# zfountas/deep-active-inference-mc

Measured on AMD Instinct MI355X. Metric: EFE rollouts/sec (64x64 dSprites, 10 MC-samples, depth 5), higher is better.
Workload: dtype f32; 1 GPU; calculate_G_repeated: 128 rows (32 roots x 4 actions) x depth 5 x 10 MC samples per GPU (BASELINE configs[1]) + action posterior; rows_per_gpu=128, samples=10, depth=5, parallelism=episodes sharded x1, weights replicated

## Files before the change

deep-active-inference-mc_amd/csrc/decoder.hip:

```cpp
#include "mfma_pipe.h"

namespace efe {

constexpr int DA_PS = 17;
constexpr int DA_BIAS = 257 * DA_PS;

__host__ __device__ constexpr int wino_i0(int a) { return a == 0 ? 0 : (a == 2 ? 2 : 1); }
__host__ __device__ constexpr int wino_i1(int a) { return a == 0 ? 2 : (a == 1 ? 2 : (a == 2 ? 1 : 3)); }
__host__ __device__ constexpr float wino_s1(int a) { return a == 1 ? 1.0f : -1.0f; }
__host__ __device__ constexpr float wino_at(int r, int a) { return r == 0 ? (a < 3 ? 1.0f : 0.0f) : (a == 0 ? 0.0f : (a == 1 ? 1.0f : -1.0f)); }

template <int NR, int R0, class Pix>
__device__ __forceinline__ void wino_l1(f32x16 (&out)[NR][2], const float4* __restrict__ U, const float4* sm, const int h,
                                        const int mt_, Pix pix) {
    constexpr int PD = 4;
    const unsigned ln = (threadIdx.x & 63u) * 16u;
    const __amdgpu_buffer_rsrc_t ur = wrsrc(U);
    int mt = mt_; asm volatile("" : "+s"(mt));
    constexpr int a_lo = NR == 2 ? 0 : R0, a_hi = NR == 2 ? 4 : R0 + 3;
    auto ufrag = [&](int a, int b, int kc) { return wfrag(ur, ln, (size_t)(((4 * a + b) * 2 + mt) * 8 + kc) * 64); };
    auto bases = [&](int a, int b, int (&pb)[4]) {
        const int i0 = wino_i0(a), i1 = wino_i1(a), j0 = wino_i0(b), j1 = wino_i1(b);
        pb[0] = pix(i0, j0); pb[1] = pix(i0, j1); pb[2] = pix(i1, j0); pb[3] = pix(i1, j1);
    };
    float4 aq[PD], raw[4];
    int pb[4];
#pragma unroll
    for (int p = 0; p < PD; ++p) aq[p] = ufrag(a_lo, 0, p);
    bases(a_lo, 0, pb);
#pragma unroll
    for (int q = 0; q < 4; ++q) raw[q] = sm[pb[q] + h];
    f32x16 xacc;
    const f32x16 zero = {};
    auto otrans = [&](int a, int b, const f32x16& m, auto mask) {
        constexpr int MASK = decltype(mask)::value;
#pragma unroll
        for (int r = 0; r < NR; ++r) {
            if (!((MASK >> r) & 1)) continue;
            const float car = wino_at(R0 + r, a);
#pragma unroll
            for (int c = 0; c < 2; ++c) {
                const float cbc = wino_at(c, b);
                if (cbc == 0.0f) continue;
                const float cf = car * cbc;
#pragma unroll
                for (int e = 0; e < 16; ++e) out[r][c][e] = __builtin_fmaf(cf, m[e], out[r][c][e]);
            }
        }
    };
    auto xi_row = [&](int a, auto mask) {
        const float s1 = wino_s1(a);
        const int an = a + 1 < a_hi ? a + 1 : a;
// ... 215 lines not shown
            return ((unsigned)y < 16u && (unsigned)x < 16u ? sy * 16 + x : DAS_IN) * DA_PS;
        };
        if (r) wino_l1<1, 1>(o, W1, sin, h, mt, pix);
        else wino_l1<1, 0>(o, W1, sin, h, mt, pix);
        if (j < 16)
#pragma unroll
        for (int c = 0; c < 2; ++c)
#pragma unroll
            for (int g4 = 0; g4 < 4; ++g4) {
                float4 v;
                v.x = relu_bits(o[0][c][4 * g4 + 0]); v.y = relu_bits(o[0][c][4 * g4 + 1]);
                v.z = relu_bits(o[0][c][4 * g4 + 2]); v.w = relu_bits(o[0][c][4 * g4 + 3]);
                sl1[((ly + 1 + r) * 16 + lx + 1 + c) * DA_PS + mt * 8 + 2 * g4 + h] = v;
            }
    }
    __syncthreads();
    float* Y = a.y2 + (size_t)img * (32 * 32 * 64);
    const int vrows = min(4, 16 - 2 * p);
#pragma unroll 1
    for (int k = 0; k < 2; ++k) {
        const int par = (w & 1) ? (k ? 2 : 1) : (k ? 3 : 0);
        const int ph = par >> 1, pw = par & 1;
        acc_init(16);
        tap_loop_pd<1, 1, 2>(acc, (1 + ph) * (1 + pw), W2, sl1, h, ConvT2Addr<1, DA_PS>{ph, pw, j >> 4, 0, j & 15, vrows, 16, DAS_L1}, PackedWIdx{2, 8, mt});
        float4* yp = reinterpret_cast<float4*>(Y) + (size_t)par * 4096 + ((2 * p) * 16 + j) * 2 + h;
#pragma unroll
        for (int g4 = 0; g4 < 4; ++g4) {
            float4 v;
            v.x = relu_bits(acc[0][0][4 * g4 + 0]); v.y = relu_bits(acc[0][0][4 * g4 + 1]);
            v.z = relu_bits(acc[0][0][4 * g4 + 2]); v.w = relu_bits(acc[0][0][4 * g4 + 3]);
            yp[(mt * 4 + g4) * 512] = v;
        }
    }
}

constexpr size_t DA_LDS_BYTES = (257 * DA_PS + 33) * sizeof(float4);
int init_dec_b_kernels();
int init_decoder_kernels() {
    if (hipFuncSetAttribute((const void*)k_dec_a, hipFuncAttributeMaxDynamicSharedMemorySize, DA_LDS_BYTES) != hipSuccess) return 1;
    if (hipFuncSetAttribute((const void*)k_dec_a_s, hipFuncAttributeMaxDynamicSharedMemorySize, DAS_LDS_BYTES) != hipSuccess) return 1;
    return init_dec_b_kernels();
}

void launch_dec_a(const DecAArgs& a, hipStream_t st) {
    if (a.parts == 8) {
        hipLaunchKernelGGL(k_dec_a_s, dim3(a.rows * 8), dim3(256), DAS_LDS_BYTES, st, a);
        return;
    }
    const size_t lds = DA_LDS_BYTES;
    const int grid = a.rows < 512 ? a.rows : 512;
    hipLaunchKernelGGL(k_dec_a, dim3(grid), dim3(256), lds, st, a);
}

template <int PARTS>
__global__ void __launch_bounds__(256, 2) k_dec_b4(const DecBArgs a) {
    constexpr int SR = 4, NW = 4, NTHR = 256;
    constexpr int DB_ZERO = (SR + 1) * 32;
    constexpr int DB_PS = 17;
    constexpr int DB_IN_F4 = (DB_ZERO + 1) * DB_PS;
    constexpr int DB_YROWS = 4 * SR + 2;
    constexpr int NPF = (SR + 1) * 512 / NTHR;
    constexpr int NS = 32 / SR;
    extern __shared__ __attribute__((aligned(16))) float4 sm[];
    float* sH = reinterpret_cast<float*>(sm + DB_IN_F4);
    __shared__ float4 sb3[8];
    const int tid = threadIdx.x;
    const int lane = tid & 63;
    const int w = __builtin_amdgcn_readfirstlane(tid >> 6);
    const int j = lane & 31, h = lane >> 5;
    constexpr int parts = PARTS;
    const int img = parts == 1 ? (int)blockIdx.x : (int)(blockIdx.x >> 2);
    const int qtr = parts == 1 ? 0 : (int)(blockIdx.x & 3);
    if (!row_live(a.live, img)) return;
    const int s_lo = parts == 1 ? 0 : (qtr ? 2 * qtr - 1 : 0);
    const int s_hi = parts == 1 ? NS : 2 * qtr + 2;

    const int mg = a.m0 + img;
    const int g = mg / a.rows_per_group;
    const int r = mg - g * a.rows_per_group;
    int gt, gp, gs;
    group_decode(a.gm, g, gt, gp, gs);
    const int mode = (gp == 0 && a.reward0) ? 1 : 0;
    const int slot = (gp == 0 && a.store0) ? gt * a.gm.S + gs : -1;
    float* po = (slot >= 0) ? a.po + ((size_t)slot * a.rows_per_group + r) * 4096 : nullptr;

    __shared__ float sq[4 * NTHR];
    __shared__ float sQ[4];
    if (tid < 8) sb3[tid] = reinterpret_cast<const float4*>(a.b3)[tid];
    __shared__ float4 sW4[8 * 12];
    if (tid < 96) {
        const int pat = tid / 12, i4 = tid - pat * 12;
        const int kw = pat & 3, hh = pat >> 2, kh = i4 >> 2, g4 = i4 & 3;
        sW4[tid] = kw < 3 ? reinterpret_cast<const float4*>(a.w4 + (3 * kh + kw) * 32)[2 * g4 + hh] : make_float4(0.f, 0.f, 0.f, 0.f);
    }
    const float4* w4p = sW4 + (h * 4 + (lane & 3)) * 12;
    if (tid < 16) sm[DB_ZERO * DB_PS + tid] = make_float4(0.f, 0.f, 0.f, 0.f);

    const float4* X = reinterpret_cast<const float4*>(a.y2) + (size_t)img * (32 * 32 * 16);
    const float4* W3 = reinterpret_cast<const float4*>(a.w3);
    const __amdgpu_buffer_rsrc_t wr = wrsrc(W3);
    const unsigned ln = (unsigned)lane * 16u;
    const float D1 = 1.00001f, D0 = 0.00001f;
    float part = 0.f;
    f32x4 pf[NPF];
    f32x4* smv = reinterpret_cast<f32x4*>(sm);
    const f32x4* Xv = reinterpret_cast<const f32x4*>(X);
    auto y2_at = [&](int iy, int idx) -> size_t { return (size_t)(((iy & 1) * 16 + ((idx & 511) >> 5)) * 512 + (iy >> 1) * 32 + (idx & 31)); };
#pragma unroll
    for (int it = 0; it < NPF; ++it) { const int idx = it * NTHR + tid; pf[it] = Xv[y2_at(min(SR * s_lo + (idx >> 9), 31), idx)]; }

    const int spA = w * 32 + j;
    const int spB = (j < 31) ? w * 32 + j + 1 : DB_ZERO;
    const int spC = (w + 1) * 32 + j;
    const int spD = (j < 31) ? (w + 1) * 32 + j + 1 : DB_ZERO;
    auto wf = [&](int tap, int kc) -> float4 { return wfrag(wr, ln, (size_t)(tap * 8 + kc) * 64); };

    constexpr int RWG = 2 * SR / NW;
    float gh[RWG][6], gpr[RWG];
    auto g_load = [&](int oh, int q, int r0y, int hb0) {
#pragma unroll
        for (int kh = 0; kh < 3; ++kh) {
            const int tr = oh + 1 - kh;
            const bool rv = tr >= 0 && tr <= 63;
            int hs = hb0 + (tr - r0y);
            hs = hs < 0 ? hs + DB_YROWS : hs;
            hs = hs >= DB_YROWS ? hs - DB_YROWS : hs;
            hs = rv ? hs : 0;
            const float* hq = sH + ((hs * 2) * 3 + kh) * 64 + lane;
            gh[q][2 * kh] = hq[0]; gh[q][2 * kh + 1] = hq[3 * 64];
        }
    };
    auto g_sig = [&](int oh, int q) {
        float v = a.b4;
#pragma unroll
        for (int kh = 0; kh < 3; ++kh) {
            const int tr = oh + 1 - kh;
            v += (tr >= 0 && tr <= 63) ? gh[q][2 * kh] + gh[q][2 * kh + 1] : 0.f;
        }
        gpr[q] = hw_sigmoid(v);
    };
    auto g_term = [&](int oh, int q) {
#pragma clang fp contract(off)
        const float pr = gpr[q];
        const float l1 = hw_log(D1 - pr), l0 = hw_log(D0 + pr);
        const float te = __builtin_fmaf(pr - 1.0f, l1, -(pr * l0));
        const float tw = reward_term(pr, oh, lane, 64, 64, a.reward_intent);
        const float t = mode == 0 ? te : tw;
        part += oh >= 0 ? t : 0.0f;
    };
    auto g_store = [&](int oh, int q) {
        if (po && oh >= 0) {
            int owl = lane; asm volatile("" : "+v"(owl));
            (po + oh * 64)[owl] = gpr[q];
        }
    };
    auto prefetch = [&](int sn, int tl) {
#pragma unroll
        for (int it = 0; it < NPF; ++it) {
            const int idx = it * NTHR + tl;
            const int grow = min(SR * sn + (idx >> 9), 31);
            pf[it] = Xv[y2_at(grow, idx)];
        }
    };

    auto fold = [&](int k) { sq[k * NTHR + tid] = part; part = 0.f; };
    int hb = 0, hbp = 0;
    for (int s = s_lo; s < s_hi; ++s) {
        const int tl = tid;
        const bool gq = parts == 1 ? true : s == 2 * qtr + 1;
        const int oh0 = 2 * SR * (s - 1) - 1 + w, oh1 = oh0 + NW;
#pragma unroll
        for (int it = 0; it < NPF; ++it) {
            const int idx = it * NTHR + tl;
            const int rl = idx >> 9, seg = (idx & 511) >> 5, wi = idx & 31;
            const int ix = 2 * (wi >> 1) + (seg >> 3), c4 = 2 * (seg & 7) + (wi & 1);
            smv[(rl * 32 + ix) * DB_PS + c4] = (SR * s + rl < 32) ? pf[it] : (f32x4)(0.f);
        }
        float4 a0 = wf(4, 0), a1 = wf(5, 0), a2 = wf(7, 0), a3 = wf(8, 0);
        __syncthreads();

        f32x16 acc[4], bias16;
#pragma unroll
        for (int g4 = 0; g4 < 4; ++g4) {
            const float4 bb = sb3[2 * g4 + h];
            bias16[4 * g4] = bb.x; bias16[4 * g4 + 1] = bb.y; bias16[4 * g4 + 2] = bb.z; bias16[4 * g4 + 3] = bb.w;
        }
        {
            float4 b = sm[spA * DB_PS + h];
#pragma unroll
            for (int kc = 0; kc < 8; ++kc) {
                const float4 c0 = a0, c1 = a1, c2 = a2, c3 = a3, cb = b;
                if (kc < 7) {
                    a0 = wf(4, kc + 1); a1 = wf(5, kc + 1); a2 = wf(7, kc + 1); a3 = wf(8, kc + 1);
                    b = sm[spA * DB_PS + 2 * (kc + 1) + h];
                } else {
                    a0 = wf(3, 0); a1 = wf(6, 0);
                    b = sm[spB * DB_PS + h];
                }
                __builtin_amdgcn_sched_barrier(0);
                if (kc == 0) { MFMA4I(acc[0], bias16, c0, cb) MFMA4I(acc[1], bias16, c1, cb) MFMA4I(acc[2], bias16, c2, cb) MFMA4I(acc[3], bias16, c3, cb) }
                else { MFMA4(acc[0], c0, cb) MFMA4(acc[1], c1, cb) MFMA4(acc[2], c2, cb) MFMA4(acc[3], c3, cb) }
                if (gq) {
                    if (kc == 0) { g_load(oh0, 0, 2 * SR * (s - 1), hbp); g_load(oh1, 1, 2 * SR * (s - 1), hbp); }
                    if (kc == 2) g_sig(oh0, 0);
                    if (kc == 4) g_term(oh0, 0);
                    if (kc == 6) g_sig(oh1, 1);
                }
            }
            float4 bd;
#pragma unroll
            for (int kc = 0; kc < 8; ++kc) {
                const float4 c0 = a0, c1 = a1, cb = b;
                if (kc < 7) {
                    a0 = wf(3, kc + 1); a1 = wf(6, kc + 1);
                    b = sm[spB * DB_PS + 2 * (kc + 1) + h];
                } else {
                    a0 = wf(1, 0); a1 = wf(2, 0); a2 = wf(0, 0);
                    b = sm[spC * DB_PS + h];
                    bd = sm[spD * DB_PS + h];
                }
                __builtin_amdgcn_sched_barrier(0);
                MFMA4(acc[1], c0, cb) MFMA4(acc[3], c1, cb)
                if (kc == 1 && gq) g_term(oh1, 1);
            }
#pragma unroll
            for (int kc = 0; kc < 8; ++kc) {
                const float4 c0 = a0, c1 = a1, c2 = a2, cb = b, cd = bd;
                if (kc < 7) {
                    a0 = wf(1, kc + 1); a1 = wf(2, kc + 1); a2 = wf(0, kc + 1);
                    b = sm[spC * DB_PS + 2 * (kc + 1) + h];
                    bd = sm[spD * DB_PS + 2 * (kc + 1) + h];
                }
                if (kc == 6) prefetch((s < NS - 1) ? s + 1 : NS - 1, tl);
                __builtin_amdgcn_sched_barrier(0);
                MFMA4(acc[3], c1, cb) MFMA4(acc[2], c0, cb) MFMA4(acc[3], c2, cd)
            }
        }
        float w4g[3][16];
#pragma unroll
        for (int i4 = 0; i4 < 12; ++i4) {
            const float4 q = w4p[i4];
            w4g[i4 >> 2][4 * (i4 & 3)] = q.x; w4g[i4 >> 2][4 * (i4 & 3) + 1] = q.y; w4g[i4 >> 2][4 * (i4 & 3) + 2] = q.z; w4g[i4 >> 2][4 * (i4 & 3) + 3] = q.w;
        }
#pragma unroll
        for (int ph = 0; ph < 2; ++ph) {
            f32x4 Tq[2][3];
#pragma unroll
            for (int e = 0; e < 16; ++e) { acc[2 * ph][e] = relu_bits(acc[2 * ph][e]); acc[2 * ph + 1][e] = relu_bits(acc[2 * ph + 1][e]); }
#pragma unroll
            for (int pw = 0; pw < 2; ++pw)
#pragma unroll
                for (int kh = 0; kh < 3; ++kh) Tq[pw][kh] = (f32x4)(0.f);
#pragma unroll
            for (int e = 0; e < 16; ++e)
#pragma unroll
                for (int kh = 0; kh < 3; ++kh) {
                    Tq[0][kh] = __builtin_amdgcn_mfma_f32_4x4x1f32(w4g[kh][e], acc[2 * ph][e], Tq[0][kh], 0, 0, 0);
                    Tq[1][kh] = __builtin_amdgcn_mfma_f32_4x4x1f32(w4g[kh][e], acc[2 * ph + 1][e], Tq[1][kh], 0, 0, 0);
                }
            int hsw = hb + 2 * w + ph;
            hsw = hsw >= DB_YROWS ? hsw - DB_YROWS : hsw;
            float* hp = sH + ((hsw * 2 + h) * 3) * 64 + 2 * j;
#pragma unroll
            for (int kh = 0; kh < 3; ++kh) {
                float l = wave_shr1(Tq[1][kh][2]), r = wave_shl1(Tq[0][kh][0]);
                l = (j == 0) ? 0.f : l;
                r = (j == 31) ? 0.f : r;
                float2 eo;
                eo.x = (Tq[1][kh][0] + Tq[0][kh][1]) + l;
                eo.y = (r + Tq[1][kh][1]) + Tq[0][kh][2];
                *reinterpret_cast<float2*>(hp + kh * 64) = eo;
            }
        }
        __syncthreads();
        if (gq) { g_store(oh0, 0); g_store(oh1, 1); }
        if (parts == 1 && (s == 2 || s == 4 || s == 6)) fold(s / 2 - 1);
        if (s == s_hi - 1) {
#pragma unroll
            for (int q = 0; q <= RWG; ++q) {
                if (q == RWG && (w != 0 || s != NS - 1)) break;
                const int oh = 2 * SR * s - 1 + q * NW + w;
                g_load(oh, 0, 2 * SR * s, hb); g_sig(oh, 0); g_term(oh, 0); g_store(oh, 0);
            }
        }
        hbp = hb;
        hb += 2 * SR;
        hb = hb >= DB_YROWS ? hb - DB_YROWS : hb;
    }
    fold(parts == 1 ? 3 : 0);
    __syncthreads();
    if (w < (parts == 1 ? 4 : 1)) {
        const float* qk = sq + w * NTHR + lane;
        float v = (qk[0] + qk[64]) + (qk[128] + qk[192]);
#pragma unroll
        for (int o = 32; o > 0; o >>= 1) v += __shfl_xor(v, o);
        if (lane == 0) sQ[w] = v;
    }
    __syncthreads();
    if (tid == 0) {
        if (parts == 1) a.val[mg] = (sQ[0] + sQ[1]) + (sQ[2] + sQ[3]);
        else a.valq[(size_t)mg * 4 + qtr] = sQ[0];
    }
}

constexpr size_t DB_LDS4D = ((5 * 32 + 1) * 17) * sizeof(float4) + 18 * 2 * 3 * 64 * sizeof(float);
int init_dec_b_kernels() {
    if (hipFuncSetAttribute((const void*)k_dec_b4<1>, hipFuncAttributeMaxDynamicSharedMemorySize, DB_LDS4D) != hipSuccess) return 1;
    if (hipFuncSetAttribute((const void*)k_dec_b4<4>, hipFuncAttributeMaxDynamicSharedMemorySize, DB_LDS4D) != hipSuccess) return 1;
    return 0;
}

void launch_dec_b(const DecBArgs& a, hipStream_t st) {
    if (a.parts == 4) hipLaunchKernelGGL(k_dec_b4<4>, dim3(a.rows * 4), dim3(256), DB_LDS4D, st, a);
    else hipLaunchKernelGGL(k_dec_b4<1>, dim3(a.rows), dim3(256), DB_LDS4D, st, a);
}

__host__ __device__ inline int fc4_spg(int mtiles) { return ((mtiles + 7) / 8 + 7) / 8; }
template <int NT>
__global__ void __launch_bounds__(256, 2) k_fc4(const GemmArgs a) {
    constexpr int RT = 32 * NT;
    extern __shared__ __attribute__((aligned(16))) float4 sm[];
    const int tid = threadIdx.x;
    const int lane = tid & 63;
    const int w = __builtin_amdgcn_readfirstlane(tid >> 6);
    const int j = lane & 31, h = lane >> 5;
    const int fgrp = blockIdx.x & 7;
    const int nper = gridDim.x >> 3, k = blockIdx.x >> 3;
    const int SPG = fc4_spg(a.mtiles);
    const int nsteps = ((a.n_pix + RT - 1) / RT) * SPG;
    const int q0 = (int)(((long)nsteps * k) / nper), q1 = (int)(((long)nsteps * (k + 1)) / nper);
    f32x4* smv = reinterpret_cast<f32x4*>(sm);
    const float4* Wl = reinterpret_cast<const float4*>(a.Wp);
    auto xaddr = [&](int t, int (&bs)[NT], int (&sw)[NT], int& wt) {
        wt = t;
#pragma unroll
        for (int nt = 0; nt < NT; ++nt) { bs[nt] = (nt * 32 + j) * 64 + t * 16; sw[nt] = j & 15; }
    };
    int cur_rt = -1;
    uint32_t krow[2] = {0, 0}, kstream[2] = {0, 0}, kstage[2] = {0, 0};
    bool rv[2] = {false, false};
#pragma unroll 1
    for (int q = q0; q < q1; ++q) {
        const int rt = q / SPG, fs = q - rt * SPG;
        const int row0 = rt * RT;
        if (rt != cur_rt) {
            if (cur_rt >= 0) __syncthreads();
            cur_rt = rt;
            const f32x4* X = reinterpret_cast<const f32x4*>(a.X);
#pragma unroll
            for (int it = 0; it < 8 * NT; ++it) {
                const int idx = it * 256 + tid;
                const int r = idx >> 6, c4 = idx & 63;
                const int gr = row0 + r;
                smv[r * 64 + (c4 ^ (r & 15))] = (gr < a.n_pix) ? X[(size_t)gr * 64 + c4] : (f32x4)(0.f);
            }
            __syncthreads();
#pragma unroll
            for (int nt = 0; nt < NT; ++nt) {
// ... 59 lines not shown
```

deep-active-inference-mc_amd/csrc/engine.hip:

```cpp
#include <hip/hip_runtime.h>
#include <algorithm>
#include <cstdio>
#include <cstring>
#include <map>
#include <mutex>
#include <string>
#include <vector>
#include "../../include/efe_engine.h"
#include "ctx_registry.h"
#include "kernels.h"

using namespace efe;

#define HIPCHK(x) do { hipError_t e_ = (x); if (e_ != hipSuccess) { return ctx->fail(std::string(#x) + ": " + hipGetErrorString(e_)); } } while (0)

namespace {

constexpr int S_DIM = 10;
constexpr int64_t MAC_TRANS = 541696, MAC_DEC = 43256320, MAC_ENC = 3868960, MAC_HABIT = 18176;

enum ProfClass { PROF_MID = 0, PROF_DEC_FC = 1, PROF_DEC_FC4 = 2, PROF_CT1 = 3, PROF_CT2 = 4, PROF_CT3 = 5, PROF_FINAL = 6,
                 PROF_ENC = 7, PROF_OTHER = 8, PROF_NCLS = 9 };

struct HostTensor { std::vector<float> data; std::vector<int64_t> shape; };
// ... 89 lines not shown
    }

    std::string pending;
    int fail(const std::string& m) { err = m; return 1; }

    void* alloc(size_t bytes) {
        bytes = (bytes + (size_t)arena_align - 1) / (size_t)arena_align * (size_t)arena_align;
        while (true) {
            if (arena.cur < arena.blocks.size()) {
                auto& b = arena.blocks[arena.cur];
                if (arena.off + bytes <= b.second) {
                    void* p = b.first + arena.off; arena.off += bytes; arena.used_total += bytes;
                    if (arena.used_total > high_water) high_water = arena.used_total;
                    return p;
                }
                arena.cur++; arena.off = 0;
                continue;
            }
            size_t sz = std::max(bytes, (size_t)256 << 20);
            char* p = nullptr;
            if (hipMalloc((void**)&p, sz) != hipSuccess) { err = "arena hipMalloc failed"; return nullptr; }
            arena.blocks.push_back({p, sz});
            ++arena_grows;
        }
    }
    template <class T> T* allocT(size_t n) { return reinterpret_cast<T*>(alloc(n * sizeof(T))); }
};

namespace {

template <class Get>
int upload_packed(efe_ctx* ctx, Layer& L, int ntaps, int cout, int cin, Get get, const float* bias_src, const int* bias_perm) {
    L.ntaps = ntaps; L.cout = cout; L.mtiles = (cout + 31) / 32; L.cin = (cin + 7) / 8 * 8;
    const int KC = L.cin / 8;
    std::vector<float> p((size_t)ntaps * L.mtiles * KC * 256);
    size_t idx = 0;
    for (int t = 0; t < ntaps; ++t)
        for (int mt = 0; mt < L.mtiles; ++mt)
            for (int kc = 0; kc < KC; ++kc)
                for (int lane = 0; lane < 64; ++lane)
                    for (int s = 0; s < 4; ++s) {
                        const int co = mt * 32 + (lane & 31), ci = kc * 8 + 4 * (lane >> 5) + s;
                        p[idx++] = (co < cout && ci < cin) ? get(t, co, ci) : 0.f;
                    }
    std::vector<float> b((size_t)L.mtiles * 32, 0.f);
    for (int co = 0; co < cout; ++co) b[co] = bias_src[bias_perm ? bias_perm[co] : co];
    HIPCHK(hipMalloc((void**)&L.Wp, p.size() * 4)); ctx->wbufs.push_back(L.Wp);
    HIPCHK(hipMalloc((void**)&L.bias, b.size() * 4)); ctx->wbufs.push_back(L.bias);
    HIPCHK(hipMemcpy(L.Wp, p.data(), p.size() * 4, hipMemcpyHostToDevice));
    HIPCHK(hipMemcpy(L.bias, b.data(), b.size() * 4, hipMemcpyHostToDevice));
    return 0;
}

const HostTensor* need(efe_ctx* ctx, const std::string& key, std::initializer_list<int64_t> shape) {
    auto it = ctx->raw.find(key);
    if (it == ctx->raw.end()) { ctx->err = "missing weight " + key; return nullptr; }
    if (it->second.shape != std::vector<int64_t>(shape)) { ctx->err = "bad shape for " + key; return nullptr; }
    return &it->second;
}

int pack_linear(efe_ctx* ctx, Layer& L, const std::string& key, int out, int in, const int* row_perm, const int* col_perm) {
    const HostTensor* w = need(ctx, key + ".weight", {out, in});
    const HostTensor* b = need(ctx, key + ".bias", {out});
    if (!w || !b) return 1;
    const float* W = w->data.data();
    return upload_packed(ctx, L, 1, out, in,
        [&](int, int co, int ci) { return W[(size_t)(row_perm ? row_perm[co] : co) * in + (col_perm ? col_perm[ci] : ci)]; },
        b->data.data(), row_perm);
}

int pack_linear16(efe_ctx* ctx, const float4*& Wout, const float*& bout, const std::string& key, int out, int in, const int* col_perm = nullptr) {
    const HostTensor* w = need(ctx, key + ".weight", {out, in});
    const HostTensor* b = need(ctx, key + ".bias", {out});
    if (!w || !b) return 1;
    const int mtiles = (out + 15) / 16, KC = (in + 15) / 16;
    std::vector<float> p((size_t)mtiles * KC * 256, 0.f), bb((size_t)mtiles * 16, 0.f);
    for (int mt = 0; mt < mtiles; ++mt)
        for (int kc = 0; kc < KC; ++kc)
            for (int lane = 0; lane < 64; ++lane)
                for (int s_ = 0; s_ < 4; ++s_) {
                    const int co = 16 * mt + (lane & 15), ci = 16 * kc + 4 * (lane >> 4) + s_;
                    if (co < out && ci < in) p[(((size_t)mt * KC + kc) * 64 + lane) * 4 + s_] = w->data[(size_t)co * in + (col_perm ? col_perm[ci] : ci)];
                }
    for (int co = 0; co < out; ++co) bb[co] = b->data[co];
    float *dW = nullptr, *dB = nullptr;
    HIPCHK(hipMalloc((void**)&dW, p.size() * 4)); ctx->wbufs.push_back(dW);
    HIPCHK(hipMalloc((void**)&dB, bb.size() * 4)); ctx->wbufs.push_back(dB);
    HIPCHK(hipMemcpy(dW, p.data(), p.size() * 4, hipMemcpyHostToDevice));
    HIPCHK(hipMemcpy(dB, bb.data(), bb.size() * 4, hipMemcpyHostToDevice));
    Wout = reinterpret_cast<const float4*>(dW); bout = dB;
    return 0;
}

struct NoiseCfg {
    uint32_t k0 = 0, k1 = 0;
    GroupMap gm{1, 1, {0, 0, 0}, 0, 0};
    int rows_per_group = 1;
    uint32_t row_offset = 0;
    const uint8_t* mask = nullptr;
    int mask_div = 1;
};
inline RowMask live_of(const NoiseCfg& nc, int m0) { return RowMask{nc.mask, nc.mask_div, m0, nc.rows_per_group, nc.mask ? nc.gm.ids : nullptr}; }

void fc(efe_ctx* ctx, const Layer& L, const float* X, int ldx, int x_mod, float* Y, int ldy, int M, bool relu, bool drop,
        uint32_t tag, const NoiseCfg& nc, int m0, hipStream_t st, bool split16 = true) {
    GemmArgs a{};
// ... 812 lines not shown
        const HostTensor* b = need(ctx, std::string(ck[i]) + ".bias", {cco[i]});
        if (!w || !b) return 1;
        const float* W = w->data.data(); const int Cin = cci[i];
        if (upload_packed(ctx, ctx->enc_conv[i], 9, cco[i], Cin,
                          [&](int t, int co, int ci) { return W[((size_t)co * Cin + ci) * 9 + t]; }, b->data.data(), nullptr)) return 1;
        if (i == 2) {
            std::vector<float> p((size_t)9 * 4 * 4 * 256);
            for (int t = 0; t < 9; ++t) for (int blk = 0; blk < 4; ++blk) for (int mt = 0; mt < 4; ++mt) for (int lane = 0; lane < 64; ++lane)
                for (int s_ = 0; s_ < 4; ++s_)
                    p[((((size_t)t * 4 + blk) * 4 + mt) * 64 + lane) * 4 + s_] = W[((size_t)(16 * mt + (lane & 15)) * 64 + 16 * blk + 4 * (lane >> 4) + s_) * 9 + t];
            HIPCHK(hipMemcpy(ctx->enc_conv[2].Wp, p.data(), p.size() * 4, hipMemcpyHostToDevice));
        }
    }
    {
        std::vector<int> colp(576);
        for (int p = 0; p < 9; ++p) for (int c = 0; c < 64; ++c) colp[p * 64 + c] = c * 9 + p;
        if (pack_linear(ctx, ctx->enc_fc[0], "down.qs_net.9", 256, 576, nullptr, colp.data())) return 1;
        if (pack_linear16(ctx, ctx->enc16.w[0], ctx->enc16.b[0], "down.qs_net.9", 256, 576, colp.data())) return 1;
        ctx->enc16_kc0 = 36;
    }
    {
        std::vector<int> rowp(16384);
        for (int p = 0; p < 256; ++p) for (int c = 0; c < 64; ++c) rowp[p * 64 + c] = c * 256 + p;
        if (pack_linear(ctx, ctx->dec_fc[3], "down.po_net.9", 16384, 256, rowp.data(), nullptr)) return 1;
        if (ctx->mfma_bf16x3 && pack_fc4_b3(ctx, (int)ctx->mfma_bf16x3)) return 1;
    }
    for (int i = 0; i < 3; ++i) {
        const HostTensor* w = need(ctx, std::string(tk[i]) + ".weight", {tci[i], tco[i], 3, 3});
        const HostTensor* b = need(ctx, std::string(tk[i]) + ".bias", {tco[i]});
        if (!w || !b) return 1;
        const float* W = w->data.data(); const int Cout = tco[i];
        if (i == 0) {
            static const double Gm[4][3] = {{1, 0, 0}, {0.5, 0.5, 0.5}, {0.5, -0.5, 0.5}, {0, 0, 1}};
            std::vector<float> U((size_t)16 * 64 * 64);
            for (int co = 0; co < 64; ++co)
                for (int ci = 0; ci < 64; ++ci) {
                    const float* k = W + ((size_t)ci * 64 + co) * 9;
                    double Gg[4][3];
                    for (int a = 0; a < 4; ++a)
                        for (int v = 0; v < 3; ++v) {
                            double s = 0;
                            for (int u = 0; u < 3; ++u) s += Gm[a][u] * (double)k[(2 - u) * 3 + (2 - v)];
                            Gg[a][v] = s;
                        }
                    for (int a = 0; a < 4; ++a)
                        for (int b = 0; b < 4; ++b) {
                            double s = 0;
                            for (int v = 0; v < 3; ++v) s += Gg[a][v] * Gm[b][v];
                            U[((size_t)(a * 4 + b) * 64 + co) * 64 + ci] = (float)s;
                        }
                }
            if (upload_packed(ctx, ctx->dec_ct[0], 16, 64, 64, [&](int t, int co, int ci) { return U[((size_t)t * 64 + co) * 64 + ci]; },
                              b->data.data(), nullptr)) return 1;
            continue;
        }
        if (upload_packed(ctx, ctx->dec_ct[i], 9, Cout, tci[i],
                          [&](int t, int co, int ci) { return W[((size_t)ci * Cout + co) * 9 + t]; }, b->data.data(), nullptr)) return 1;
    }
    {
        const HostTensor* w = need(ctx, "down.po_net.19.weight", {32, 1, 3, 3});
        const HostTensor* b = need(ctx, "down.po_net.19.bias", {1});
        if (!w || !b) return 1;
        std::vector<float> wf(288);
        for (int t = 0; t < 9; ++t) for (int ci = 0; ci < 32; ++ci) wf[t * 32 + ci] = w->data[ci * 9 + t];
        HIPCHK(hipMalloc((void**)&ctx->dec_wf, 288 * 4)); ctx->wbufs.push_back(ctx->dec_wf);
        HIPCHK(hipMemcpy(ctx->dec_wf, wf.data(), 288 * 4, hipMemcpyHostToDevice));
        ctx->dec_bf = b->data[0];
    }
    ctx->committed = true;
    return 0;
}

int efe_env_reset(efe_ctx* ctx, float* state, float* last_r, int E, const efe_noise* nz, void* stream) {
    Call call(ctx, Mode::device); if (!call) return 1;
    if (!state || !last_r || !nz || E < 1) return ctx->fail("efe_env_reset: bad arguments");
    launch_env_reset(state, last_r, E, (uint32_t)nz->seed, (uint32_t)(nz->seed >> 32), nz->stage, nz->row_offset, (hipStream_t)stream);
    return call.finish();
}

int efe_env_new_image(efe_ctx* ctx, float* state, int E, const efe_noise* nz, void* stream) {
    Call call(ctx, Mode::device); if (!call) return 1;
    if (!state || !nz || E < 1) return ctx->fail("efe_env_new_image: bad arguments");
    launch_env_new_image(state, E, (uint32_t)nz->seed, (uint32_t)(nz->seed >> 32), nz->stage, nz->row_offset, (hipStream_t)stream);
    return call.finish();
}

int efe_env_step(efe_ctx* ctx, float* state, float* last_r, const int32_t* actions, int E, int repeats, const efe_noise* nz,
                 int32_t* round_changed, void* stream) {
    Call call(ctx, Mode::device); if (!call) return 1;
    if (!state || !last_r || !actions || !nz || E < 1 || repeats < 1) return ctx->fail("efe_env_step: bad arguments");
    launch_env_step(state, last_r, actions, round_changed, E, repeats, (uint32_t)nz->seed, (uint32_t)(nz->seed >> 32), nz->stage,
                    nz->row_offset, (hipStream_t)stream);
    return call.finish();
}

int efe_env_render(efe_ctx* ctx, const float* state, const float* last_r, const uint8_t* imgs, int64_t n_imgs, float* frames,
                   int32_t* err, int E, void* stream) {
    Call call(ctx, Mode::device); if (!call) return 1;
    if (!state || !last_r || !imgs || !frames || n_imgs < 1 || E < 1) return ctx->fail("efe_env_render: bad arguments");
    launch_env_render(state, last_r, imgs, (long)n_imgs, frames, err, E, (hipStream_t)stream);
    return call.finish();
}

int efe_mcts_select(efe_ctx* ctx, const efe_mcts_tree* tree, const uint8_t* active, float C, int use_prior, int max_depth,
                    int32_t* path_nodes, int32_t* path_act, int32_t* path_len, int32_t* leaf, float* leaf_s, float* leaf_s_rep,
                    void* stream) {
// ... 498 lines not shown
```

deep-active-inference-mc_amd/csrc/kernels.h:

```cpp
#pragma once
#include <hip/hip_runtime.h>
#include <stdint.h>
#include "philox.h"

namespace efe {

struct GroupMap {
    int per_stage, S;
    uint32_t pass[3];
    uint32_t stage0, sample0;
    const int32_t* ids = nullptr; int ids_div = 1;
};
__device__ __forceinline__ uint32_t global_row(const int32_t* ids, int ids_div, int r, uint32_t row_offset) {
    if (!ids) return row_offset + (uint32_t)r;
    const int e = r / ids_div;
    return row_offset + (uint32_t)(ids[e] * ids_div + (r - e * ids_div));
}
__host__ __device__ inline void group_decode(const GroupMap& gm, int g, int& t, int& pidx, int& samp) {
    t = g / gm.per_stage;
    const int q = g - t * gm.per_stage;
    pidx = q / gm.S;
    samp = q - pidx * gm.S;
}
__device__ __forceinline__ uint2 group_key(const GroupMap& gm, int g) {
// ... 7 lines not shown
    const uint8_t* mask; int div, m0, rows_per_group;
    const int32_t* ids = nullptr;
};
__device__ __forceinline__ bool row_live(const RowMask& k, int m) {
    if (!k.mask) return true;
    const int slot = ((k.m0 + m) % k.rows_per_group) / k.div;
    return k.mask[k.ids ? k.ids[slot] : slot] != 0;
}

__device__ __forceinline__ float reward_term(float pr, int oh, int ow, int H, int W, int intent) {
#pragma clang fp contract(off)
    const float D1 = 1.00001f, D0 = 0.00001f;
    const bool one = intent ? (ow < W / 2) : (oh < H / 2);
    const float t = one ? __builtin_fmaf(pr, logf(D1), (1.0f - pr) * logf(D1 - 1.0f)) : __builtin_fmaf(pr, logf(D0), (1.0f - pr) * logf(D1));
    return (intent && oh >= 3) ? 0.0f : t;
}

struct GemmArgs {
    const float* Wp;
    const float* bias;
    const float* X;
    float* Y;
    const float* zeros;
    int n_pix;
    int cin;
    int cout;
    int mtiles;
    int ldx, ldy;
    int x_mod;
    int relu;
    int dropout;
    uint32_t tag, k0, k1;
    GroupMap gm;
    int rows_per_group;
    uint32_t row_offset;
    int m0;
    const void* Wb3 = nullptr;
    int split = 0;
    float wb3_scale_inv = 1.0f;
};

struct DecAArgs {
    const float* x4; float* y2;
    const float* w1; const float* b1;
    const float* w2; const float* b2;
    int rows;
    RowMask live;
    int parts;
    int* queue;
    const void* w1b3 = nullptr; const void* w2b3 = nullptr;
    int split = 0;
    float w1s = 1.0f, w1s_inv = 1.0f, w2s = 1.0f, w2s_inv = 1.0f;
};
struct DecBArgs {
    const float* y2;
    const float* w3; const float* b3;
    const float* w4; float b4;
    int rows;
    RowMask live;
    int m0;
    int rows_per_group;
    GroupMap gm;
    int reward0;
    int store0;
    float* val;
    int parts;
    float* valq;
    float* po;
    int reward_intent;
    const void* w3b3 = nullptr;
    int split = 0;
    float w3s = 1.0f, w3s_inv = 1.0f;
};
struct EncArgs {
    const float* o; float* out;
    const float* w1; const float* b1;
    const float* w2; const float* b2;
    const float* w3; const float* b3;
    const float* w4; const float* b4;
    int rows;
    RowMask live;
};
void launch_enc_trunk(const EncArgs& a, hipStream_t st);
void launch_fc4(const GemmArgs& a, hipStream_t st);
void launch_fc4_b3(const GemmArgs& a, hipStream_t st);
float pack_dense_split(int mode, const float* W, const int* row_perm, int out, int in, uint16_t* dst);
void launch_dec_a_b3(const DecAArgs& a, hipStream_t st);
float pack_conv_split(int mode, const float* W_cicokk, int Cin, int Cout, uint16_t* dst);
void launch_dec_b_b3(const DecBArgs& a, hipStream_t st);
float pack_convt3_split(int mode, const float* W_cicokk, uint16_t* dst);
int init_bf16x3_kernels();
void launch_dec_a(const DecAArgs& a, hipStream_t st);
void launch_dec_b(const DecBArgs& a, hipStream_t st);

int launch_dense(int MT, int NT, const GemmArgs& a, hipStream_t st);

struct TransPostArgs {
    const float* tr;
    const float* x;
    const float* eps_inj;
    const float* given_ps1;
    float* dec_in;
    float* next_x;
    float* ps1_last;
    float* ps1_mean_last;
    int S, R, mean_mode, carry_mean;
// ... 200 lines not shown
```

Measured before the change: 10600 rollouts/s.

## Rewrite dec_b stride-2 transposed conv as fast-algorithm 2x2 tile with 16x16x4 MFMA

Replaces the direct 9-tap transposed-convolution in the dec_b kernel with a Winograd-like F(2x2) transform. Input views are linear combinations of neighbouring pixels, host-precomputed transformed weights (16 matrices) are repacked per half-channel, and products are scattered into 16 output-phase accumulators via constexpr-scheduled 16x16x4 MFMAs. The final 32->1 conv also moves to 16x16x4 MFMA with DPP shifts. The intent is fewer multiplies and better MFMA shape. The cost is higher register pressure, a changed LDS padding layout, and more complex compile-time scheduling.

```diff
diff --git a/deep-active-inference-mc_amd/csrc/decoder.hip b/deep-active-inference-mc_amd/csrc/decoder.hip
--- a/deep-active-inference-mc_amd/csrc/decoder.hip
+++ b/deep-active-inference-mc_amd/csrc/decoder.hip
@@ -1,3 +1,4 @@
+#include <utility>
 #include "mfma_pipe.h"
 
 namespace efe {
@@ -319,22 +320,58 @@
     hipLaunchKernelGGL(k_dec_a, dim3(grid), dim3(256), lds, st, a);
 }
 
+template <class F, int... I> __device__ __forceinline__ void static_for_(F&& f, std::integer_sequence<int, I...>) { (f(std::integral_constant<int, I>{}), ...); }
+template <int N, class F> __device__ __forceinline__ void static_for(F&& f) { static_for_(f, std::make_integer_sequence<int, N>{}); }
+
+__host__ __device__ constexpr int w3_nch(int G) { return G == 4 ? 5 : 4; }
+__host__ __device__ constexpr int w3_prod(int G, int c) {
+    return G < 4 ? 5 * ((G >> 1) + 2 * (c >> 1)) + (G & 1) + 2 * (c & 1)
+         : G == 4 ? (c < 2 ? 5 * (1 + 2 * c) + 4 : c < 4 ? 20 + 1 + 2 * (c - 2) : 24)
+                  : (c < 2 ? 5 * (2 * c) + 4 : 20 + 2 * (c - 2));
+}
+__host__ __device__ constexpr bool w3_direct(int pp) { return f22_o1(pp / 5) < 0 && f22_o1(pp % 5) < 0; }
+__host__ __device__ constexpr int w3_view(int pp) { return 3 * f22_view(pp / 5) + f22_view(pp % 5); }
+__host__ __device__ constexpr int w3_mat(int pp) { return 4 * f22_wt(pp / 5) + f22_wt(pp % 5); }
+__host__ __device__ constexpr bool w3_hits(int pp, int o) {
+    const int r = o >> 2, c = o & 3, pr = pp / 5, pc = pp % 5;
+    return (r == f22_o0(pr) || r == f22_o1(pr)) && (c == f22_o0(pc) || c == f22_o1(pc));
+}
+__host__ __device__ constexpr bool w3_seen(int G, int c, int o) {
+    for (int g = 0; g < G; ++g)
+        for (int k = 0; k < w3_nch(g); ++k) if (w3_hits(w3_prod(g, k), o)) return true;
+    if (!w3_direct(w3_prod(G, c)))
+        for (int k = 0; k < w3_nch(G); ++k)
+            if ((w3_direct(w3_prod(G, k)) || k < c) && w3_hits(w3_prod(G, k), o)) return true;
+    return false;
+}
+__host__ __device__ constexpr bool w3_uses_view(int G, int vi) {
+    for (int k = 0; k < w3_nch(G); ++k) if (w3_view(w3_prod(G, k)) == vi) return true;
+    return false;
+}
+__host__ __device__ constexpr bool f22_in(int a, int r) { return a == 0 ? r <= 1 : (a == 1 ? r == 1 : r >= 1); }
+__host__ __device__ constexpr bool w3_reads(int G, int r, int c) {
+    for (int vi = 0; vi < 9; ++vi) if (w3_uses_view(G, vi) && f22_in(vi / 3, r) && f22_in(vi % 3, c)) return true;
+    return false;
+}
+
 template <int PARTS>
 __global__ void __launch_bounds__(256, 2) k_dec_b4(const DecBArgs a) {
     constexpr int SR = 4, NW = 4, NTHR = 256;
-    constexpr int DB_ZERO = (SR + 1) * 32;
+    constexpr int DB_RP = 33;
     constexpr int DB_PS = 17;
-    constexpr int DB_IN_F4 = (DB_ZERO + 1) * DB_PS;
+    constexpr int DB_IN_F4 = (SR + 1) * DB_RP * DB_PS;
     constexpr int DB_YROWS = 4 * SR + 2;
     constexpr int NPF = (SR + 1) * 512 / NTHR;
     constexpr int NS = 32 / SR;
+    constexpr int NST = 24;
     extern __shared__ __attribute__((aligned(16))) float4 sm[];
     float* sH = reinterpret_cast<float*>(sm + DB_IN_F4);
     __shared__ float4 sb3[8];
     const int tid = threadIdx.x;
     const int lane = tid & 63;
     const int w = __builtin_amdgcn_readfirstlane(tid >> 6);
-    const int j = lane & 31, h = lane >> 5;
+    const int g = lane >> 4, v = lane & 15;
+    const int u = w >> 1, hf = w & 1;
     constexpr int parts = PARTS;
     const int img = parts == 1 ? (int)blockIdx.x : (int)(blockIdx.x >> 2);
     const int qtr = parts == 1 ? 0 : (int)(blockIdx.x & 3);
@@ -343,10 +380,10 @@
     const int s_hi = parts == 1 ? NS : 2 * qtr + 2;
 
     const int mg = a.m0 + img;
-    const int g = mg / a.rows_per_group;
-    const int r = mg - g * a.rows_per_group;
+    const int gi = mg / a.rows_per_group;
+    const int r = mg - gi * a.rows_per_group;
     int gt, gp, gs;
-    group_decode(a.gm, g, gt, gp, gs);
+    group_decode(a.gm, gi, gt, gp, gs);
     const int mode = (gp == 0 && a.reward0) ? 1 : 0;
     const int slot = (gp == 0 && a.store0) ? gt * a.gm.S + gs : -1;
     float* po = (slot >= 0) ? a.po + ((size_t)slot * a.rows_per_group + r) * 4096 : nullptr;
@@ -354,19 +391,18 @@
     __shared__ float sq[4 * NTHR];
     __shared__ float sQ[4];
     if (tid < 8) sb3[tid] = reinterpret_cast<const float4*>(a.b3)[tid];
-    __shared__ float4 sW4[8 * 12];
-    if (tid < 96) {
-        const int pat = tid / 12, i4 = tid - pat * 12;
-        const int kw = pat & 3, hh = pat >> 2, kh = i4 >> 2, g4 = i4 & 3;
-        sW4[tid] = kw < 3 ? reinterpret_cast<const float4*>(a.w4 + (3 * kh + kw) * 32)[2 * g4 + hh] : make_float4(0.f, 0.f, 0.f, 0.f);
-    }
-    const float4* w4p = sW4 + (h * 4 + (lane & 3)) * 12;
-    if (tid < 16) sm[DB_ZERO * DB_PS + tid] = make_float4(0.f, 0.f, 0.f, 0.f);
+    if (tid < (SR + 1) * 16) sm[((tid >> 4) * DB_RP + 32) * DB_PS + (tid & 15)] = make_float4(0.f, 0.f, 0.f, 0.f);
+    f32x4 w4a;
+    {
+        const int kh = v >> 2, kw = v & 3;
+#pragma unroll
+        for (int rr = 0; rr < 4; ++rr) w4a[rr] = (kh < 3 && kw < 3) ? a.w4[(3 * kh + kw) * 32 + 16 * hf + 4 * g + rr] : 0.f;
+    }
 
     const float4* X = reinterpret_cast<const float4*>(a.y2) + (size_t)img * (32 * 32 * 16);
-    const float4* W3 = reinterpret_cast<const float4*>(a.w3);
-    const __amdgpu_buffer_rsrc_t wr = wrsrc(W3);
+    const __amdgpu_buffer_rsrc_t wr = wrsrc(a.w3 + (size_t)hf * 4 * 64 * 4);
     const unsigned ln = (unsigned)lane * 16u;
+    auto wf = [&](int m, int kc) -> f32x4 { return __builtin_bit_cast(f32x4, wfrag(wr, ln, (size_t)(m * 8 + kc) * 64)); };
     const float D1 = 1.00001f, D0 = 0.00001f;
     float part = 0.f;
     f32x4 pf[NPF];
@@ -376,11 +412,13 @@
 #pragma unroll
     for (int it = 0; it < NPF; ++it) { const int idx = it * NTHR + tid; pf[it] = Xv[y2_at(min(SR * s_lo + (idx >> 9), 31), idx)]; }
 
-    const int spA = w * 32 + j;
-    const int spB = (j < 31) ? w * 32 + j + 1 : DB_ZERO;
-    const int spC = (w + 1) * 32 + j;
-    const int spD = (j < 31) ? (w + 1) * 32 + j + 1 : DB_ZERO;
-    auto wf = [&](int tap, int kc) -> float4 { return wfrag(wr, ln, (size_t)(tap * 8 + kc) * 64); };
+    const int xb = (2 * u * DB_RP + 2 * v) * DB_PS + g;
+    auto px = [&](int i, int jj, int kc) -> f32x4 { return smv[xb + (i * DB_RP + jj) * DB_PS + 4 * kc]; };
+    auto view = [&](const f32x4 (&x)[9], int vi) -> f32x4 {
+        const int va = vi / 3, vb = vi % 3;
+        auto cv = [&](int i) -> f32x4 { return vb == 0 ? x[3 * i] - x[3 * i + 1] : (vb == 1 ? x[3 * i + 1] : x[3 * i + 2] - x[3 * i + 1]); };
+        return va == 0 ? cv(0) - cv(1) : (va == 1 ? cv(1) : cv(2) - cv(1));
+    };
 
     constexpr int RWG = 2 * SR / NW;
     float gh[RWG][6], gpr[RWG];
@@ -398,13 +436,13 @@
         }
     };
     auto g_sig = [&](int oh, int q) {
-        float v = a.b4;
+        float val = a.b4;
 #pragma unroll
         for (int kh = 0; kh < 3; ++kh) {
             const int tr = oh + 1 - kh;
-            v += (tr >= 0 && tr <= 63) ? gh[q][2 * kh] + gh[q][2 * kh + 1] : 0.f;
-        }
-        gpr[q] = hw_sigmoid(v);
+            val += (tr >= 0 && tr <= 63) ? gh[q][2 * kh] + gh[q][2 * kh + 1] : 0.f;
+        }
+        gpr[q] = hw_sigmoid(val);
     };
     auto g_term = [&](int oh, int q) {
 #pragma clang fp contract(off)
@@ -433,7 +471,7 @@
     auto fold = [&](int k) { sq[k * NTHR + tid] = part; part = 0.f; };
     int hb = 0, hbp = 0;
     for (int s = s_lo; s < s_hi; ++s) {
-        const int tl = tid;
+        int tl = tid; asm volatile("" : "+v"(tl));
         const bool gq = parts == 1 ? true : s == 2 * qtr + 1;
         const int oh0 = 2 * SR * (s - 1) - 1 + w, oh1 = oh0 + NW;
 #pragma unroll
@@ -441,103 +479,82 @@
             const int idx = it * NTHR + tl;
             const int rl = idx >> 9, seg = (idx & 511) >> 5, wi = idx & 31;
             const int ix = 2 * (wi >> 1) + (seg >> 3), c4 = 2 * (seg & 7) + (wi & 1);
-            smv[(rl * 32 + ix) * DB_PS + c4] = (SR * s + rl < 32) ? pf[it] : (f32x4)(0.f);
-        }
-        float4 a0 = wf(4, 0), a1 = wf(5, 0), a2 = wf(7, 0), a3 = wf(8, 0);
+            smv[(rl * DB_RP + ix) * DB_PS + c4] = (SR * s + rl < 32) ? pf[it] : (f32x4)(0.f);
+        }
+        f32x4 aq[5];
+#pragma unroll
+        for (int c = 0; c < w3_nch(0); ++c) aq[c] = wf(w3_mat(w3_prod(0, c)), 0);
         __syncthreads();
 
-        f32x16 acc[4], bias16;
-#pragma unroll
-        for (int g4 = 0; g4 < 4; ++g4) {
-            const float4 bb = sb3[2 * g4 + h];
-            bias16[4 * g4] = bb.x; bias16[4 * g4 + 1] = bb.y; bias16[4 * g4 + 2] = bb.z; bias16[4 * g4 + 3] = bb.w;
-        }
-        {
-            float4 b = sm[spA * DB_PS + h];
-#pragma unroll
-            for (int kc = 0; kc < 8; ++kc) {
-                const float4 c0 = a0, c1 = a1, c2 = a2, c3 = a3, cb = b;
-                if (kc < 7) {
-                    a0 = wf(4, kc + 1); a1 = wf(5, kc + 1); a2 = wf(7, kc + 1); a3 = wf(8, kc + 1);
-                    b = sm[spA * DB_PS + 2 * (kc + 1) + h];
-                } else {
-                    a0 = wf(3, 0); a1 = wf(6, 0);
-                    b = sm[spB * DB_PS + h];
-                }
-                __builtin_amdgcn_sched_barrier(0);
-                if (kc == 0) { MFMA4I(acc[0], bias16, c0, cb) MFMA4I(acc[1], bias16, c1, cb) MFMA4I(acc[2], bias16, c2, cb) MFMA4I(acc[3], bias16, c3, cb) }
-                else { MFMA4(acc[0], c0, cb) MFMA4(acc[1], c1, cb) MFMA4(acc[2], c2, cb) MFMA4(acc[3], c3, cb) }
-                if (gq) {
-                    if (kc == 0) { g_load(oh0, 0, 2 * SR * (s - 1), hbp); g_load(oh1, 1, 2 * SR * (s - 1), hbp); }
-                    if (kc == 2) g_sig(oh0, 0);
-                    if (kc == 4) g_term(oh0, 0);
-                    if (kc == 6) g_sig(oh1, 1);
-                }
-            }
-            float4 bd;
-#pragma unroll
-            for (int kc = 0; kc < 8; ++kc) {
-                const float4 c0 = a0, c1 = a1, cb = b;
-                if (kc < 7) {
-                    a0 = wf(3, kc + 1); a1 = wf(6, kc + 1);
-                    b = sm[spB * DB_PS + 2 * (kc + 1) + h];
-                } else {
-                    a0 = wf(1, 0); a1 = wf(2, 0); a2 = wf(0, 0);
-                    b = sm[spC * DB_PS + h];
-                    bd = sm[spD * DB_PS + h];
-                }
-                __builtin_amdgcn_sched_barrier(0);
-                MFMA4(acc[1], c0, cb) MFMA4(acc[3], c1, cb)
-                if (kc == 1 && gq) g_term(oh1, 1);
-            }
-#pragma unroll
-            for (int kc = 0; kc < 8; ++kc) {
-                const float4 c0 = a0, c1 = a1, c2 = a2, cb = b, cd = bd;
-                if (kc < 7) {
-                    a0 = wf(1, kc + 1); a1 = wf(2, kc + 1); a2 = wf(0, kc + 1);
-                    b = sm[spC * DB_PS + 2 * (kc + 1) + h];
-                    bd = sm[spD * DB_PS + 2 * (kc + 1) + h];
-                }
-                if (kc == 6) prefetch((s < NS - 1) ? s + 1 : NS - 1, tl);
-                __builtin_amdgcn_sched_barrier(0);
-                MFMA4(acc[3], c1, cb) MFMA4(acc[2], c0, cb) MFMA4(acc[3], c2, cd)
-            }
-        }
-        float w4g[3][16];
-#pragma unroll
-        for (int i4 = 0; i4 < 12; ++i4) {
-            const float4 q = w4p[i4];
-            w4g[i4 >> 2][4 * (i4 & 3)] = q.x; w4g[i4 >> 2][4 * (i4 & 3) + 1] = q.y; w4g[i4 >> 2][4 * (i4 & 3) + 2] = q.z; w4g[i4 >> 2][4 * (i4 & 3) + 3] = q.w;
-        }
-#pragma unroll
-        for (int ph = 0; ph < 2; ++ph) {
-            f32x4 Tq[2][3];
-#pragma unroll
-            for (int e = 0; e < 16; ++e) { acc[2 * ph][e] = relu_bits(acc[2 * ph][e]); acc[2 * ph + 1][e] = relu_bits(acc[2 * ph + 1][e]); }
-#pragma unroll
-            for (int pw = 0; pw < 2; ++pw)
-#pragma unroll
-                for (int kh = 0; kh < 3; ++kh) Tq[pw][kh] = (f32x4)(0.f);
-#pragma unroll
-            for (int e = 0; e < 16; ++e)
-#pragma unroll
-                for (int kh = 0; kh < 3; ++kh) {
-                    Tq[0][kh] = __builtin_amdgcn_mfma_f32_4x4x1f32(w4g[kh][e], acc[2 * ph][e], Tq[0][kh], 0, 0, 0);
-                    Tq[1][kh] = __builtin_amdgcn_mfma_f32_4x4x1f32(w4g[kh][e], acc[2 * ph + 1][e], Tq[1][kh], 0, 0, 0);
-                }
-            int hsw = hb + 2 * w + ph;
+        const f32x4 bias4 = __builtin_bit_cast(f32x4, sb3[4 * hf + g]);
+        const f32x4 zero4 = {};
+        f32x4 acc[16], tq[5];
+        f32x4 xr[9];
+        static_for<9>([&](auto i) { if constexpr (w3_reads(0, i / 3, i % 3)) xr[i] = px(i / 3, i % 3, 0); });
+        static_for<NST>([&](auto stc) {
+            constexpr int ST = decltype(stc)::value, G = ST >> 2, KC = ST & 3, GN = (ST + 1) >> 2, KN = (ST + 1) & 3;
+            f32x4 vw[9], ac[5];
+            static_for<9>([&](auto vi) { if constexpr (w3_uses_view(G, vi)) vw[vi] = view(xr, vi); });
+#pragma unroll
+            for (int c = 0; c < 5; ++c) ac[c] = aq[c];
+            if constexpr (ST + 1 < NST) {
+                static_for<w3_nch(GN)>([&](auto c) { aq[c] = wf(w3_mat(w3_prod(GN, c)), KN); });
+                static_for<9>([&](auto i) { if constexpr (w3_reads(GN, i / 3, i % 3)) xr[i] = px(i / 3, i % 3, KN); });
+            }
+            __builtin_amdgcn_sched_barrier(0);
+#pragma unroll
+            for (int e = 0; e < 4; ++e)
+                static_for<w3_nch(G)>([&](auto c) {
+                    constexpr int PP = w3_prod(G, c);
+                    const float b = vw[w3_view(PP)][e], av = ac[c][e];
+                    if constexpr (w3_direct(PP)) {
+                        constexpr int O = 4 * f22_o0(PP / 5) + f22_o0(PP % 5);
+                        constexpr bool FIRST = KC == 0 && !w3_seen(G, c, O);
+                        acc[O] = __builtin_amdgcn_mfma_f32_16x16x4f32(av, b, (FIRST && e == 0) ? bias4 : acc[O], 0, 0, 0);
+                    } else {
+                        tq[c] = __builtin_amdgcn_mfma_f32_16x16x4f32(av, b, (KC == 0 && e == 0) ? zero4 : tq[c], 0, 0, 0);
+                    }
+                });
+            if constexpr (KC == 3)
+                static_for<w3_nch(G)>([&](auto c) {
+                    constexpr int PP = w3_prod(G, c);
+                    if constexpr (!w3_direct(PP))
+                        static_for<16>([&](auto o) {
+                            if constexpr (w3_hits(PP, o)) {
+                                if constexpr (w3_seen(G, c, o)) acc[o] = acc[o] + tq[c];
+                                else acc[o] = bias4 + tq[c];
+                            }
+                        });
+                });
+            if (gq) {
+                if constexpr (ST == 0) { g_load(oh0, 0, 2 * SR * (s - 1), hbp); g_load(oh1, 1, 2 * SR * (s - 1), hbp); }
+                if constexpr (ST == 2) g_sig(oh0, 0);
+                if constexpr (ST == 5) g_term(oh0, 0);
+                if constexpr (ST == 8) g_sig(oh1, 1);
+                if constexpr (ST == 11) g_term(oh1, 1);
+            }
+        });
+        prefetch((s < NS - 1) ? s + 1 : NS - 1, tl);
+#pragma unroll
+        for (int orow = 0; orow < 4; ++orow) {
+            f32x4 T[4];
+#pragma unroll
+            for (int oc = 0; oc < 4; ++oc)
+#pragma unroll
+                for (int e = 0; e < 4; ++e) acc[4 * orow + oc][e] = relu_bits(acc[4 * orow + oc][e]);
+#pragma unroll
+            for (int e = 0; e < 4; ++e)
+#pragma unroll
+                for (int oc = 0; oc < 4; ++oc)
+                    T[oc] = __builtin_amdgcn_mfma_f32_16x16x4f32(w4a[e], acc[4 * orow + oc][e], e == 0 ? zero4 : T[oc], 0, 0, 0);
+            f32x4 hv;
+            hv[0] = (T[1][0] + T[0][1]) + dpp_shr1_zero(T[3][2]);
+            hv[1] = (T[2][0] + T[1][1]) + T[0][2];
+            hv[2] = (T[3][0] + T[2][1]) + T[1][2];
+            hv[3] = (dpp_shl1_zero(T[0][0]) + T[3][1]) + T[2][2];
+            int hsw = hb + 4 * u + orow;
             hsw = hsw >= DB_YROWS ? hsw - DB_YROWS : hsw;
-            float* hp = sH + ((hsw * 2 + h) * 3) * 64 + 2 * j;
-#pragma unroll
-            for (int kh = 0; kh < 3; ++kh) {
-                float l = wave_shr1(Tq[1][kh][2]), r = wave_shl1(Tq[0][kh][0]);
-                l = (j == 0) ? 0.f : l;
-                r = (j == 31) ? 0.f : r;
-                float2 eo;
-                eo.x = (Tq[1][kh][0] + Tq[0][kh][1]) + l;
-                eo.y = (r + Tq[1][kh][1]) + Tq[0][kh][2];
-                *reinterpret_cast<float2*>(hp + kh * 64) = eo;
-            }
+            if (g < 3) *reinterpret_cast<f32x4*>(sH + ((hsw * 2 + hf) * 3 + g) * 64 + 4 * v) = hv;
         }
         __syncthreads();
         if (gq) { g_store(oh0, 0); g_store(oh1, 1); }
@@ -558,10 +575,10 @@
     __syncthreads();
     if (w < (parts == 1 ? 4 : 1)) {
         const float* qk = sq + w * NTHR + lane;
-        float v = (qk[0] + qk[64]) + (qk[128] + qk[192]);
-#pragma unroll
-        for (int o = 32; o > 0; o >>= 1) v += __shfl_xor(v, o);
-        if (lane == 0) sQ[w] = v;
+        float val = (qk[0] + qk[64]) + (qk[128] + qk[192]);
+#pragma unroll
+        for (int o = 32; o > 0; o >>= 1) val += __shfl_xor(val, o);
+        if (lane == 0) sQ[w] = val;
     }
     __syncthreads();
     if (tid == 0) {
@@ -570,7 +587,7 @@
     }
 }
 
-constexpr size_t DB_LDS4D = ((5 * 32 + 1) * 17) * sizeof(float4) + 18 * 2 * 3 * 64 * sizeof(float);
+constexpr size_t DB_LDS4D = ((5 * 33) * 17) * sizeof(float4) + 18 * 2 * 3 * 64 * sizeof(float);
 int init_dec_b_kernels() {
     if (hipFuncSetAttribute((const void*)k_dec_b4<1>, hipFuncAttributeMaxDynamicSharedMemorySize, DB_LDS4D) != hipSuccess) return 1;
     if (hipFuncSetAttribute((const void*)k_dec_b4<4>, hipFuncAttributeMaxDynamicSharedMemorySize, DB_LDS4D) != hipSuccess) return 1;
diff --git a/deep-active-inference-mc_amd/csrc/engine.hip b/deep-active-inference-mc_amd/csrc/engine.hip
--- a/deep-active-inference-mc_amd/csrc/engine.hip
+++ b/deep-active-inference-mc_amd/csrc/engine.hip
@@ -165,6 +165,21 @@
     return 0;
 }
 
+std::vector<float> convt_s2_f22_weights(const float* W, int cin, int cout) {
+    std::vector<float> U((size_t)16 * cout * cin);
+    for (int wr = 0; wr < 4; ++wr)
+        for (int wc = 0; wc < 4; ++wc)
+            for (int co = 0; co < cout; ++co)
+                for (int ci = 0; ci < cin; ++ci) {
+                    const float* k = W + ((size_t)ci * cout + co) * 9;
+                    double s = 0;
+                    for (int kh = 0; kh < 3; ++kh)
+                        for (int kw = 0; kw < 3; ++kw) s += (double)(f22_cw(wr, kh) * f22_cw(wc, kw)) * (double)k[kh * 3 + kw];
+                    U[((size_t)(4 * wr + wc) * cout + co) * cin + ci] = (float)s;
+                }
+    return U;
+}
+
 const HostTensor* need(efe_ctx* ctx, const std::string& key, std::initializer_list<int64_t> shape) {
     auto it = ctx->raw.find(key);
     if (it == ctx->raw.end()) { ctx->err = "missing weight " + key; return nullptr; }
@@ -1083,6 +1098,16 @@
                 }
             if (upload_packed(ctx, ctx->dec_ct[0], 16, 64, 64, [&](int t, int co, int ci) { return U[((size_t)t * 64 + co) * 64 + ci]; },
                               b->data.data(), nullptr)) return 1;
+            continue;
+        }
+        if (i == 2) {
+            const std::vector<float> U = convt_s2_f22_weights(W, 64, 32);
+            if (upload_packed(ctx, ctx->dec_ct[2], 16, 32, 64, [](int, int, int) { return 0.f; }, b->data.data(), nullptr)) return 1;
+            std::vector<float> p(U.size());
+            for (int m = 0; m < 16; ++m) for (int hf = 0; hf < 2; ++hf) for (int kc = 0; kc < 4; ++kc) for (int lane = 0; lane < 64; ++lane)
+                for (int s_ = 0; s_ < 4; ++s_)
+                    p[((((size_t)m * 2 + hf) * 4 + kc) * 64 + lane) * 4 + s_] = U[((size_t)m * 32 + 16 * hf + (lane & 15)) * 64 + 16 * kc + 4 * (lane >> 4) + s_];
+            HIPCHK(hipMemcpy(ctx->dec_ct[2].Wp, p.data(), p.size() * 4, hipMemcpyHostToDevice));
             continue;
         }
         if (upload_packed(ctx, ctx->dec_ct[i], 9, Cout, tci[i],
diff --git a/deep-active-inference-mc_amd/csrc/kernels.h b/deep-active-inference-mc_amd/csrc/kernels.h
--- a/deep-active-inference-mc_amd/csrc/kernels.h
+++ b/deep-active-inference-mc_amd/csrc/kernels.h
@@ -83,6 +83,12 @@
     int split = 0;
     float w1s = 1.0f, w1s_inv = 1.0f, w2s = 1.0f, w2s_inv = 1.0f;
 };
+__host__ __device__ constexpr int f22_view(int p) { return p == 4 ? 2 : (p & 1); }
+__host__ __device__ constexpr int f22_wt(int p) { return p < 2 ? 0 : p - 1; }
+__host__ __device__ constexpr int f22_o0(int p) { return p < 2 ? 0 : (p < 4 ? 1 : 3); }
+__host__ __device__ constexpr int f22_o1(int p) { return p == 1 ? 2 : (p == 3 ? 3 : -1); }
+__host__ __device__ constexpr int f22_cw(int wt, int k) { return wt == 0 ? (k == 1) : wt == 1 ? (k == 2) : wt == 2 ? (k != 1) : (k == 0); }
+
 struct DecBArgs {
     const float* y2;
     const float* w3; const float* b3;
```

New measurement: 11270 rollouts/s, median of 6. 1.06x the previous value.
